# MattiaDallaCosta/JPEG-encoder-decoder

Measured on AMD Instinct MI355X. Metric: Mpixels/s encoded (device-resident BGR888 -> JFIF bytes), higher is better.
Workload: dtype int8-MFMA exact + fp64 replay (bit-exact); 1 GPU; config 3: 256 x 3840x2160 BGR888 frames per GPU, 4:2:0, Q=50, one independent JFIF per frame; frames_per_gpu=256, width=3840, height=2160, quality=50, mode=encode, pipeline=fused, parallelism=frame-parallel x1

## Files before the change

### jpeg-encoder-decoder_amd/csrc/mij_api.hip

```cpp
#include <math.h>
#include <stdarg.h>
#include <string.h>

#include <mutex>
#include <vector>

#include "mij_host.h"
#include "mij_internal.h"
#include "mij_interleave.h"
#include "mij_sampled.h"
#include "mij_ijg.h"
#include "mij_transcode.h"
#include "mijpeg.h"
#include "mij_testing.h"

namespace mij {
int k1_grid(int device, long long ntiles, int mode);
hipError_t launch_colour_lut(uint32_t *lut, hipStream_t s);
hipError_t launch_k1(const K1Args &a, int grid, int mode, hipStream_t s);
hipError_t launch_fix_blocks(const K1Args &a, hipStream_t s);
hipError_t launch_seg_dc(const EntArgs &a, hipStream_t s);
hipError_t launch_segdc_actab(const EntArgs &a, hipStream_t s);
hipError_t launch_dc_diff(int16_t *coef, const int16_t *dc, const Geom &g, int nframes,
                          const int2 *fd, hipStream_t s);
// ... 286 lines not shown
  bool assembler = false;
  std::vector<unsigned long long> band_words;
  int band_async_n = 0;
  int asm_tables_n = 0;
  int hist_zero_n = 0;
  int band_hist_zero = 0;
  int hist_zero_after = 0;
  unsigned long long *d_bound_acc = nullptr;
  int2 *d_fdims = nullptr;
  int4 *d_regions = nullptr;
  bool use_fdims = false;
  std::vector<int2> h_fdims;
  uint8_t *d_frame = nullptr;
  size_t frame_cap = 0;
  int raw_dirty = 0;
  bool keep_coefs = false;
  bool rgb = false;
  bool split = false;
  int overlap = 1;
  hipStream_t stream2 = nullptr;
  hipEvent_t ov_k1[16] = {}, ov_done = nullptr;
  bool timing = false;
  int k1_err_zero = 0;
  int opt[MIJ_OPT_COUNT] = {1, 1, 1, 0, -1, 0, 1, 0, -1};
  static constexpr int HIST = 64;
  hipEvent_t evh[HIST][MIJ_NSTAGES] = {};
  hipEvent_t *ev = evh[0];
  long long steps = 0;
  int last_frames = 0;
  int plan[MIJ_PLAN_FIELDS] = {};
  std::vector<int4> il_slot;
  long long out_cap0 = 0;
  int2 *d_il_tdims = nullptr;
  uint16_t *d_il_blk_bits = nullptr;
  uint32_t *d_il_mcu_off = nullptr, *d_il_row_bits = nullptr, *d_il_ffc = nullptr;
  uint64_t *d_il_row_pre = nullptr, *d_il_ival = nullptr, *d_il_row_off = nullptr;
  int *d_il_hdr = nullptr;
  struct DevBuf {
    void *p = nullptr;
    size_t bytes = 0;
  };
  enum { SB_PLANE, SB_ABS, SB_FR, SB_TFR, SB_TOUT, SB_BLK_BITS, SB_MCU_OFF, SB_ROW_BITS, SB_ROW_PRE, SB_IVAL,
         SB_ROW_OFF, SB_BITS, SB_HDR, SB_RAW, SB_FFC, SB_IJGQ, SB_COUNT };
  DevBuf sb[SB_COUNT];
  int samp_last = -1;
  int samp_n = 0, samp_rr = 0;
// ... 4 lines not shown
  std::vector<SampFrame> h_sfr;
  std::vector<TcFrame> h_stf;
  std::vector<TcOut> h_sto;
  int samp_test_frame = -1;
  long long samp_test_cap = 0;
};

template <class T>
static hipError_t dalloc(T **p, size_t count) {
  return hipMalloc((void **)p, count * sizeof(T) + 256);
}

static void batch_free(mij_batch *b) {
  if (!b) return;
  hipSetDevice(b->dev);
  if (b->own_stream && b->stream != b->own_stream) {
    if (b->stream && b->ev_switch && hipEventRecord(b->ev_switch, b->stream) == hipSuccess)
      hipStreamWaitEvent(b->own_stream, b->ev_switch, 0);
    b->stream = b->own_stream;
  }
  if (b->own_stream) hipStreamSynchronize(b->own_stream);
  void *ptrs[] = {b->d_tab, b->own_in ? b->d_in : nullptr, b->d_coef, b->d_dc, b->d_hist,
                  b->d_ehuf, b->d_raw, b->d_tok, b->d_tok0, b->d_seg_ntok, b->d_seg_bits, b->d_seg_off,
                  b->d_scan_bits, b->d_out_len, b->d_hc, b->d_out, b->d_err, b->d_replays,
                  b->d_dcpred, b->d_bitbase, b->d_stage, b->d_fixmask, b->d_audit, b->d_ffc, b->d_choff, b->d_scan_base,
                  b->d_seam, b->d_pack_state, b->d_pack_ticket, b->d_fdims, b->d_frame, b->d_regions, b->d_pieces,
                  b->d_bound_acc, b->d_dcx, b->d_il_tdims, b->d_il_blk_bits, b->d_il_mcu_off, b->d_il_row_bits,
                  b->d_il_ffc, b->d_il_row_pre, b->d_il_ival, b->d_il_row_off, b->d_il_hdr};
  for (void *p : ptrs)
    if (p) hipFree(p);
  for (mij_batch::DevBuf &d : b->sb)
    if (d.p) hipFree(d.p);
  for (auto &row : b->evh)
    for (auto &e : row)
      if (e) hipEventDestroy(e);
  for (auto &e : b->ov_k1)
    if (e) hipEventDestroy(e);
  if (b->ov_done) hipEventDestroy(b->ov_done);
  if (b->stream2) {
    hipStreamSynchronize(b->stream2);
    hipStreamDestroy(b->stream2);
  }
  if (b->ev_switch) hipEventDestroy(b->ev_switch);
  if (b->own_stream) hipStreamDestroy(b->own_stream);
  delete b;
}

// ... 45 lines not shown
    HIP_TRY(hipMemsetAsync(b->d_fixmask, 0, sizeof(uint16_t) * F * g.tiles_per_frame * 3, b->stream));
    HIP_TRY(dalloc(&b->d_pack_state, F * pack_stride(g)));
    HIP_TRY(dalloc(&b->d_pack_ticket, F * 3));
    HIP_TRY(dalloc(&b->d_dcx, F * 64));
    HIP_TRY(hipMemsetAsync(b->d_dcx, 0, sizeof(uint32_t) * F * 64, b->stream));
    HIP_TRY(dalloc(&b->d_seam, F * pack_stride(g)));
    HIP_TRY(dalloc(&b->d_regions, F));
  }
  HIP_TRY(dalloc(&b->d_hist, F * 4 * 257));
  HIP_TRY(dalloc(&b->d_ehuf, F * 4 * 256));
  HIP_TRY(dalloc(&b->d_raw, F * g.raw_fs));
  HIP_TRY(hipMemsetAsync(b->d_raw, 0, sizeof(uint32_t) * F * g.raw_fs, b->stream));
  HIP_TRY(dalloc(&b->d_scan_bits, F * 3));
  HIP_TRY(dalloc(&b->d_out_len, F));
  HIP_TRY(dalloc(&b->d_hc, F * 4));
  HIP_TRY(dalloc(&b->d_out, F * g.out_cap));
  HIP_TRY(dalloc(&b->d_err, F));
  HIP_TRY(dalloc(&b->d_replays, 1));
  HIP_TRY(dalloc(&b->d_ffc, F * 3 * emit_chunks(g)));
  HIP_TRY(dalloc(&b->d_choff, F * 3 * emit_chunks(g)));
  HIP_TRY(dalloc(&b->d_scan_base, F * 3));
  HIP_TRY(hipMemsetAsync(b->d_ffc, 0, sizeof(uint32_t) * F * 3 * emit_chunks(g), b->stream));
  HIP_TRY(hipMemsetAsync(b->d_replays, 0, sizeof(unsigned), b->stream));
  HIP_TRY(dalloc(&b->d_fdims, F));
  b->h_fdims.assign((size_t)F, make_int2(w, h));
  HIP_TRY(dalloc(&b->d_dcpred, F * 4));
  HIP_TRY(dalloc(&b->d_bitbase, F * 4));
  HIP_TRY(hipMemsetAsync(b->d_dcpred, 0, sizeof(int16_t) * F * 4, b->stream));
  HIP_TRY(hipMemsetAsync(b->d_bitbase, 0, sizeof(uint32_t) * F * 4, b->stream));
  b->band_words.assign((size_t)F * 3, 0);
  for (auto &row : b->evh)
    for (auto &e : row) HIP_TRY(hipEventCreate(&e));
  HIP_TRY(hipStreamSynchronize(b->stream));
  return MIJ_OK;
}

extern "C" mij_batch *mij_batch_create(int device, int width, int height, int max_frames,
                                       int quality) {
  if (!valid_dims(width, height) || max_frames < 1 || quality < 1 || quality > 100) {
    fail(MIJ_EINVAL, "batch_create: bad geometry %dx%d x%d or quality %d", width, height,
         max_frames, quality);
    return nullptr;
  }
  mij_batch *b = new mij_batch;
  if (batch_init(b, device, width, height, max_frames, quality)) {
    batch_free(b);
// ... 167 lines not shown
    a.seg_ntok += F * g.nseg;
    a.seg_bits += F * g.nseg;
    a.seg_off += F * g.nseg;
    a.scan_bits += F * 3;
    a.raw += F * g.raw_fs;
    a.hc += F * 4;
    a.out += F * g.out_cap;
    a.out_len += F;
    a.err += F;
    if (a.dc_pred) a.dc_pred += F * 4;
    if (a.bit_base) a.bit_base += F * 4;
    a.ffc += F * 3 * emit_chunks(g);
    a.choff += F * 3 * emit_chunks(g);
    a.scan_base += F * 3;
    a.pack_state += F * gpf;
    a.pack_ticket += F * 3;
    if (a.dcx) a.dcx += F * 64;
    if (a.fdims) a.fdims += F;
  }
  return a;
}

static int run_k1(mij_batch *b, int nframes, int mode, int dc_diffed = 0, int seg_dc_inline = 0, int f0 = 0,
                  bool stage_events = true, bool dc_only = false) {
  if (mode & 2) b->hist_zero_n = b->band_hist_zero = 0;
  K1Args k;
  memset(&k, 0, sizeof(k));
  k.in = b->d_in;
  k.in_fs = b->in_fs;
  k.pitch = b->pitch;
  k.nframes = nframes;
  k.g = b->g;
  k.coef = b->d_coef;
  k.dc = b->d_dc;
  k.tab = b->d_tab;
  k.replays = b->d_replays;
  k.tok = b->d_tok;
  k.tok0 = b->d_tok0;
  k.seg_ntok = b->d_seg_ntok;
  k.hist = b->d_hist;
  k.fix_mask = b->d_fixmask;
  k.audit = b->audit && mode == 1 ? b->d_audit : nullptr;
  k.rgb = b->rgb && (mode & 4) == 0;
  k.fdims = b->use_fdims ? b->d_fdims : nullptr;
  if (b->k1_err_zero) {
    k.err_zero = b->d_err;
    k.nerr_zero = b->k1_err_zero;
    b->k1_err_zero = 0;
  }
  if (f0) {
    const Geom &g = b->g;
    const long long F = f0;
    k.in += F * b->in_fs;
    k.coef += F * g.coef_fs;
    k.dc += F * g.nblk;
    k.tok += F * g.nseg * SEG_TOK;
    k.tok0 += F * g.nseg;
    k.seg_ntok += F * g.nseg;
    k.hist += F * 4 * 257;
    if (k.fdims) k.fdims += F;
  }
  static const int k1_flags = diag_env("MIJ_K1_FLAGS", 0);
  k.flags = k1_flags;
  const long long ntiles = (long long)nframes * b->g.tiles_per_frame;
  long long grid = k1_grid(b->dev, ntiles, mode);
  long long per_wg = (ntiles + grid - 1) / grid;
  if (per_wg > b->g.tiles_per_frame) per_wg = b->g.tiles_per_frame;
  grid = (ntiles + per_wg - 1) / per_wg;
  k.per_wg = (int)per_wg;
  k.dc_diffed = dc_diffed;
  k.seg_dc_inline = seg_dc_inline;
  static const bool wtime = diag_env("MIJ_K1_WTIME", 0) != 0;
  unsigned long long *d_wt = nullptr;
  const long long nw = grid * 16;
  if (wtime && (mode == 1 || mode == 2)) {
    HIP_TRY(hipMalloc(&d_wt, sizeof(unsigned long long) * K1_WTIME_WORDS * nw));
    HIP_TRY(hipMemsetAsync(d_wt, 0, sizeof(unsigned long long) * K1_WTIME_WORDS * nw, b->stream));
    k.wtime = d_wt;
  }
  k.dc_only = dc_only;
  b->plan[MIJ_PLAN_K1_MODE] = mode;
  b->plan[MIJ_PLAN_DC_ONLY] = dc_only;
  HIP_TRY(launch_k1(k, (int)grid, mode, b->stream));
  if (d_wt) {
    const int WW = K1_WTIME_WORDS;
    std::vector<unsigned long long> h(WW * nw);
    HIP_TRY(hipMemcpyAsync(h.data(), d_wt, sizeof(unsigned long long) * WW * nw, hipMemcpyDeviceToHost, b->stream));
    HIP_TRY(hipStreamSynchronize(b->stream));
    HIP_TRY(hipFree(d_wt));
    unsigned long long s0 = ~0ull, e1 = 0, e0 = ~0ull;
    double sum = 0, smin = 1e30, smax = 0, ph[5] = {0, 0, 0, 0, 0};
    long long n = 0, tiles = 0;
// ... 190 lines not shown
  if (t) HIP_TRY(hipEventRecord(b->ev[6], st));
  HIP_TRY(launch_emit(a, st));
  if (t) HIP_TRY(hipEventRecord(b->ev[7], st));
  return MIJ_OK;
}

static int encode_frames(mij_batch *b, int nframes) {
  b->plan[MIJ_PLAN_ENTROPY_CALLS] = 0;
  b->plan[MIJ_PLAN_HIST_FILL_SKIPPED] = nframes <= b->hist_zero_n;
  if (nframes > b->hist_zero_n)
    HIP_TRY(hipMemsetAsync(b->d_hist, 0, sizeof(uint32_t) * nframes * 4 * 257, b->stream));
  b->hist_zero_n = 0;
  if (b->use_fdims && b->rgb) return fail(MIJ_EINVAL, "encode: region batches read B, G, R frames");
  if (b->use_fdims)
    HIP_TRY(hipMemsetAsync(b->d_seg_ntok, 0, sizeof(uint32_t) * nframes * b->g.nseg, b->stream));
  b->k1_err_zero = nframes;
  if (b->timing) HIP_TRY(hipEventRecord(b->ev[0], b->stream));
  const bool dc_only = !b->split && !b->use_fdims && !ent_args_pack_wide(b);
  const int nsub = std::min(b->overlap, nframes);
  if (!b->split && !b->keep_coefs && nsub > 1) {
    const int per = (nframes + nsub - 1) / nsub;
    for (int k = 0, f0 = 0; f0 < nframes; k++, f0 += per) {
      const int nk = std::min(per, nframes - f0);
      if (run_k1(b, nk, 2, 0, 0, f0, false, dc_only)) return g_err;
      HIP_TRY(hipEventRecord(b->ov_k1[k], b->stream));
      HIP_TRY(hipStreamWaitEvent(b->stream2, b->ov_k1[k], 0));
      if (run_entropy(b, nk, true, false, f0, b->stream2)) return g_err;
    }
    if (b->timing)
      for (int e = 1; e <= 3; e++) HIP_TRY(hipEventRecord(b->ev[e], b->stream));
    HIP_TRY(hipEventRecord(b->ov_done, b->stream2));
    HIP_TRY(hipStreamWaitEvent(b->stream, b->ov_done, 0));
    if (b->timing)
      for (int e = 4; e < MIJ_NSTAGES; e++) HIP_TRY(hipEventRecord(b->ev[e], b->stream));
    return MIJ_OK;
  }
  if (b->split) {
    if (run_k1(b, nframes, 1)) return g_err;
    if (run_k1(b, nframes, 6, 0, 1)) return g_err;
  } else {
    if (run_k1(b, nframes, b->keep_coefs ? 3 : 2, 0, 0, 0, true, dc_only)) return g_err;
  }
  if (b->timing) HIP_TRY(hipEventRecord(b->ev[3], b->stream));
  if (run_entropy(b, nframes, !b->split, false)) return g_err;
  b->hist_zero_n = b->hist_zero_after;
  return MIJ_OK;
}

static void next_slot(mij_batch *b) {
  if (b->timing) b->ev = b->evh[b->steps++ % mij_batch::HIST];
}

extern "C" int mij_batch_encode(mij_batch *b, int nframes) {
  if (pipe_check(b, "encode")) return g_err;
  if (nframes < 1 || nframes > b->cap) return fail(MIJ_EINVAL, "encode: bad frame count");
  HIP_TRY(hipSetDevice(b->dev));
  next_slot(b);
  if (encode_frames(b, nframes)) return g_err;
  b->last_frames = nframes;
  return MIJ_OK;
}

extern "C" int mij_batch_keep_coefs(mij_batch *b, int on) {
  if (pipe_check(b, "keep_coefs")) return g_err;
// ... 558 lines not shown
    if (err[i]) return mij_frame_fail(err[i], "mij_encode_regions: region", i);
  size_t off = 0;
  for (int i = 0; i < n; i++) {
    lens[i] = len[i];
    if (off + len[i] > cap) return fail(MIJ_ENOSPC, "mij_encode_regions: need more than %zu bytes", cap);
    HIP_TRY(hipMemcpyAsync(out + off, b->d_out + (long long)i * b->g.out_cap, len[i], hipMemcpyDeviceToHost,
                           b->stream));
    off += len[i];
  }
  HIP_TRY(hipStreamSynchronize(b->stream));
  return MIJ_OK;
}

extern "C" int mij_test_last_plan(mij_batch *b, int *out, int n) {
  if (!out || n < 0) return fail(MIJ_EINVAL, "test_last_plan: bad args"), -2;
  std::unique_lock<std::mutex> l(g_mu, std::defer_lock);
  if (!b) {
    l.lock();
    b = g_rctx;
  }
  if (!b) return fail(MIJ_EINVAL, "test_last_plan: no batch"), -2;
  for (int i = 0; i < n && i < MIJ_PLAN_FIELDS; i++) out[i] = b->plan[i];
  return MIJ_PLAN_FIELDS;
}

static int band_check(mij_batch *b, int n, const char *what, bool assembling = false) {
  if (!b || n < 1 || n > b->cap) return fail(MIJ_EINVAL, "%s: bad frame count", what);
  if (!assembling && pipe_check(b, what)) return g_err;
  HIP_TRY(hipSetDevice(b->dev));
  return MIJ_OK;
}

extern "C" int mij_band_analyze(mij_batch *b, int n, int16_t *last_dc) {
  if (band_check(b, n, "band_analyze")) return g_err;
  if (!last_dc) return fail(MIJ_EINVAL, "band_analyze: null last_dc");
  HIP_TRY(hipMemsetAsync(b->d_hist, 0, sizeof(uint32_t) * n * 4 * 257, b->stream));
  HIP_TRY(hipMemsetAsync(b->d_err, 0, sizeof(int) * n, b->stream));
  if (run_k1(b, n, 2)) return g_err;
  const Geom &g = b->g;
  const long long last[3] = {g.nY - 1, g.nY + g.nC - 1, g.nY + 2LL * g.nC - 1};
  for (int c = 0; c < 3; c++)
    HIP_TRY(hipMemcpy2DAsync(last_dc + c, 3 * sizeof(int16_t), b->d_dc + last[c], sizeof(int16_t) * g.nblk,
                             sizeof(int16_t), n, hipMemcpyDeviceToHost, b->stream));
  HIP_TRY(hipStreamSynchronize(b->stream));
  return MIJ_OK;
}
// ... 1064 lines not shown
```

### jpeg-encoder-decoder_amd/csrc/mij_internal.h

```cpp
#pragma once
#include <hip/hip_runtime.h>
#include <stddef.h>
#include <stdint.h>

#include "mij_divmagic.h"

namespace mij {

constexpr int TILE_W = 128;
constexpr int TILE_H = 16;
constexpr int LDS_BLK = 80;
constexpr int LDS_WAVE = 48 * LDS_BLK;
constexpr int LUT_WORDS = 1024;
constexpr int DCTIE_WORDS = 33;

constexpr int FERR_TABLE = 1;
constexpr int FERR_OVERFLOW = 2;
constexpr int FERR_ASSEMBLY = 3;
constexpr int OPT_TEST_FAULT_TICKET = 7;
constexpr int FERR_SPIN = 4;
constexpr unsigned long long SPIN_TICKS = 200000000ull;

constexpr int MAX_BLOCK_TOK = 65;
constexpr int SEG_TOK = 16 * MAX_BLOCK_TOK;
// ... 86 lines not shown
  int nframes;
  Geom g;
  int16_t *coef;
  int16_t *dc;
  const Tables *tab;
  unsigned int *replays;
  int flags;
  int per_wg;
  int dc_diffed;
  int seg_dc_inline;
  const int16_t *dc_pred;
  uint32_t *tok;
  uint32_t *tok0;
  uint32_t *seg_ntok;
  uint32_t *hist;
  uint16_t *fix_mask;
  unsigned long long *wtime;
  int rgb;
  const int2 *fdims;
  uint16_t *audit;
  int *err_zero;
  int nerr_zero;
  int dc_only;
};
constexpr int K1_WTIME_WORDS = 8;
constexpr int K1F_NO_LUT = 1, K1F_NO_REPLAY = 2, K1F_NO_COLOUR = 4, K1F_NO_DCT = 8,
              K1F_NO_STORE = 16, K1F_NO_QUANT = 32, K1F_NO_MFMA = 64,
              K1F_LINEAR_STORE = 128, K1F_PLAIN_STORE = 256,
              K1F_NO_HIST = 512, K1F_NO_TOKSTORE = 1024,
              K1F_EXTRA_LDS = 2048, K1F_NO_EMIT = 4096, K1F_NO_ACLOOP = 8192,
              K1F_NO_DMAWAIT = 16384,
              K1F_REPLAY_NO_FP64 = 32768,
              K1F_COUNT_PASSES = 65536,
              K1F_COUNT_LUMA = 131072;

struct EntArgs {
  Geom g;
  int nframes;
  const int16_t *coef;
  const int16_t *dc;
  uint32_t *hist;
  const uint32_t *ehuf;
  uint32_t *tok;
  uint32_t *tok0;
  const uint32_t *seg_ntok;
  uint32_t *seg_bits;
  uint64_t *seg_off;
// ... 50 lines not shown
```

### jpeg-encoder-decoder_amd/csrc/mij_kernels.hip

```cpp
#include <stdlib.h>

#include "mij_internal.h"
#include "mij_headers.h"
#include "mij_colour_f64.h"

namespace mij {

typedef int v4i __attribute__((ext_vector_type(4)));
typedef unsigned u4v __attribute__((ext_vector_type(4)));
typedef unsigned short us2 __attribute__((ext_vector_type(2)));

__constant__ int c_zigzag[64] = {
    0,  1,  8,  16, 9,  2,  3,  10, 17, 24, 32, 25, 18, 11, 4,  5,
    12, 19, 26, 33, 40, 48, 41, 34, 27, 20, 13, 6,  7,  14, 21, 28,
    35, 42, 49, 56, 57, 50, 43, 36, 29, 22, 15, 23, 30, 37, 44, 51,
    58, 59, 52, 45, 38, 31, 39, 46, 53, 60, 61, 54, 47, 55, 62, 63};

#define SQRT1_2 0.70710678118654752440

__device__ __forceinline__ void wave_lds_sync() {
  __builtin_amdgcn_fence(__ATOMIC_RELEASE, "wavefront");
  __builtin_amdgcn_wave_barrier();
  __builtin_amdgcn_fence(__ATOMIC_ACQUIRE, "wavefront");
}
// ... 481 lines not shown
      const uint32_t bef = __builtin_amdgcn_ubfe(Mhi, 0u, (uint32_t)zz);
      uint32_t lz;
      asm("v_ffbh_u32 %0, %1" : "=v"(lz) : "v"(bef));
      token(32 + zz, rank_lo1 + __popc(bef), (int)min(lz, (uint32_t)(63 - zp_lo)));
    }
  }
  wave_lds_sync();
}

constexpr int K1M_COEF_OUT = 1;
constexpr int K1M_TOK_OUT = 2;
constexpr int K1M_COEF_IN = 4;
constexpr int K1M_RGB = 8;
constexpr int K1M_REGIONS = 16;
constexpr int K1M_AUDIT = 32;
constexpr int K1M_FLOOR = 64;
constexpr int k1_base(int mode) { return mode & ~(K1M_RGB | K1M_REGIONS | K1M_AUDIT | K1M_FLOOR); }

template <int MODE>
constexpr bool k1_wide() { return k1_base(MODE) == K1M_COEF_OUT || k1_base(MODE) == K1M_TOK_OUT; }
template <int MODE>
constexpr int k1_waves() {
  return k1_wide<MODE>() ? 12 : 4;
}

template <int MODE>
__global__ __launch_bounds__(64 * k1_waves<MODE>(), k1_wide<MODE>() ? 1 : 2) void k_mcu_dct(K1Args a) {
  constexpr bool PIX = !(MODE & K1M_COEF_IN);
  constexpr bool TOK = MODE & K1M_TOK_OUT;
  constexpr int NW = k1_waves<MODE>();
  constexpr int NT = 64 * NW;
  constexpr bool DEFER = k1_base(MODE) == K1M_COEF_OUT;
  constexpr bool RGB = MODE & K1M_RGB;
  constexpr bool REG = MODE & K1M_REGIONS;
  constexpr bool AUDIT = MODE & K1M_AUDIT;
  constexpr bool FLOOR = MODE & K1M_FLOOR;
  const int2 *const fdims = REG ? a.fdims : nullptr;
  __shared__ __attribute__((aligned(16))) uint8_t s_raw[PIX ? NW : 1][TILE_RAW];
  __shared__ __attribute__((aligned(16))) uint8_t s_tile[PIX ? NW : 1][LDS_WAVE];
  __shared__ __attribute__((aligned(16))) int4 s_A[PIX ? 12 * 64 : 1];
  __shared__ __attribute__((aligned(16))) float s_fac[2][64];
  __shared__ float s_inv8q[2];
  __shared__ uint32_t s_dctie[2][DCTIE_WORDS];
  constexpr bool LUT_LDS = PIX && !(TOK && NW >= 8);
  __shared__ uint32_t s_lut[LUT_LDS ? 3 * LUT_WORDS : 1];
  __shared__ double s_cos[64];
  __shared__ uint8_t s_zz[64];
  __shared__ int s_qint[2][64];
  __shared__ __attribute__((aligned(16))) int s_czl[PIX ? 64 : 1];
  __shared__ __attribute__((aligned(16))) int16_t s_st[TOK ? NW : 1][64][16];
  constexpr int HREP = PIX ? 1 : 4;
  __shared__ uint32_t s_hac[TOK ? 2 : 1][2][HREP][256];
  __shared__ uint32_t s_hdc[TOK ? 2 : 1][2][HREP][16];
  __shared__ int s_next;

  const Tables *__restrict__ T = a.tab;
#ifdef MIJ_K1_DIAG
  const int kflags = a.flags;
#else
  constexpr int kflags = 0;
#endif
  if (threadIdx.x < 64) {
    s_cos[threadIdx.x] = T->cosd[threadIdx.x];
    s_zz[threadIdx.x] = (uint8_t)c_zigzag[threadIdx.x];
  }
  if (TOK) {
    for (int i = threadIdx.x; i < 2 * 2 * HREP * 256; i += NT) (&s_hac[0][0][0][0])[i] = 0;
    for (int i = threadIdx.x; i < 2 * 2 * HREP * 16; i += NT) (&s_hdc[0][0][0][0])[i] = 0;
  }
  if (threadIdx.x < 128) s_qint[threadIdx.x >> 6][threadIdx.x & 63] = T->qint[threadIdx.x >> 6][threadIdx.x & 63];
  if (threadIdx.x < 2) s_inv8q[threadIdx.x] = 1.0f / (float)(8 * T->qint[threadIdx.x][0]);
  if (PIX && threadIdx.x < 64) s_czl[threadIdx.x] = T->czl[threadIdx.x];
  if (threadIdx.x < 2 * DCTIE_WORDS) (&s_dctie[0][0])[threadIdx.x] = (&T->dctie[0][0])[threadIdx.x];
  if (PIX) {
    for (int i = threadIdx.x; i < 12 * 64; i += NT) s_A[i] = T->mfma_a[i];
    if (LUT_LDS)
      for (int i = threadIdx.x; i < 3 * LUT_WORDS; i += NT) s_lut[i] = (&T->lut[0][0])[i];
  }
  const uint32_t *__restrict__ lut = LUT_LDS ? (const uint32_t *)s_lut : &T->lut[0][0];
  for (int i = threadIdx.x; i < 128; i += NT) {
    s_fac[i >> 6][i & 63] = T->qfac[i >> 6][i & 63];
  }
  if (threadIdx.x == 0) s_next = (int)blockIdx.x * a.per_wg + NW;
  if (blockIdx.x == 0)
    for (int i = threadIdx.x; i < a.nerr_zero; i += NT) a.err_zero[i] = 0;
  __syncthreads();

  const int lane = threadIdx.x & 63;
  const int wave = __builtin_amdgcn_readfirstlane(threadIdx.x >> 6);
  uint8_t *L = s_tile[PIX ? wave : 0];
  const int g = lane >> 4, bcol = lane & 15;
  const int c4 = lane & 31, pr = lane >> 5;
  const uint32_t kq = (uint32_t)T->kq[g];
  const int q_dc[2] = {T->qint[0][0], T->qint[1][0]};
  const bool cz_on = PIX && !AUDIT && T->cz_on;
  const Geom &G = a.g;
  const int bw = G.w >> 3, mw = G.w >> 4;
  const int ntiles = a.nframes * G.tiles_per_frame;
  const int t0 = (int)blockIdx.x * a.per_wg;
  const int f0 = t0 / G.tiles_per_frame;
  const int tend = min(ntiles, t0 + a.per_wg);
  int t = t0 + wave;
  auto skip_outside = [&](int &tt) {
    bool ok;
    while (tt < tend && (tile_pos_r(G, fdims, tt, ok), !ok)) {
      int v = 0;
      if (lane == 0) v = atomicAdd(&s_next, 1);
      tt = __builtin_amdgcn_readfirstlane(v);
    }
  };
  auto tpos = [&](int tt) {
    bool ok;
    return REG ? tile_pos_r(G, fdims, tt, ok) : tile_pos(G, tt);
  };
  if (REG) skip_outside(t);
#ifdef MIJ_K1_DIAG
  const unsigned long long w_t0 = __builtin_amdgcn_s_memrealtime();
  int w_ntiles = 0;
  unsigned long long ph[5] = {0, 0, 0, 0, 0}, tph = __builtin_amdgcn_s_memtime();
#define K1_PHASE(k)                                                  \
  do {                                                               \
    const unsigned long long tn_ = __builtin_amdgcn_s_memtime();     \
    ph[k] += tn_ - tph;                                              \
    tph = tn_;                                                       \
  } while (0)
#else
#define K1_PHASE(k)
#endif
  uint32_t nrep = 0;
  if (t < tend) {
    uint8_t *raw = s_raw[PIX ? wave : 0];
    TilePos p = tpos(t);
    const DmaOff doff = dma_offsets(a.pitch, lane);
    if (PIX) issue_tile_dma(a, p, lane, raw, doff);
    auto load_coefs = [&](const TilePos &pp, u4v (&dst)[PIX ? 1 : 3][2]) {
#pragma unroll
      for (int nt = 0; nt < 3; nt++) {
        bool valid;
        long long blk;
        const FGeom fg = frame_geom(G, fdims, pp.f);
        const int bwf = REG ? fg.bw : bw, mwf = REG ? fg.mw : mw;
        const int nYf = REG ? fg.nY : G.nY, nCf = REG ? fg.nC : G.nC;
        if (nt < 2) {
          const int bx = pp.tx * 16 + bcol;
          valid = bx < bwf;
          blk = (long long)(2 * pp.ty + nt) * bwf + bx;
        } else {
          const int mx = pp.tx * 8 + (bcol & 7);
          valid = mx < mwf;
          blk = nYf + (bcol >= 8 ? nCf : 0) + (long long)pp.ty * mwf + mx;
        }
        dst[PIX ? 0 : nt][0] = dst[PIX ? 0 : nt][1] = u4v{0, 0, 0, 0};
        if (valid) {
          const int16_t *src = a.coef + (long long)pp.f * G.coef_fs + blk * 64 + 16 * g;
          dst[PIX ? 0 : nt][0] = *(const u4v *)src;
          dst[PIX ? 0 : nt][1] = *(const u4v *)(src + 8);
        }
      }
    };
    u4v cnext[PIX ? 1 : 3][2];
    if (!PIX) load_coefs(p, cnext);
    bool first = true;
    for (;;) {
      TilePos pn = p;
      int tn = 0;
      if (lane == 0) tn = atomicAdd(&s_next, 1);
      tn = __builtin_amdgcn_readfirstlane(tn);
      uint32_t fl_w = 0;
      if (PIX) {
        K1_PHASE(3);
        if (first || (kflags & (K1F_NO_DCT | K1F_NO_STORE)))
          dma_wait();
        else if (DEFER)
          dma_wait_behind_stores();
        K1_PHASE(0);
        if (!(kflags & K1F_NO_COLOUR) && !FLOOR) colour_stage<RGB, !LUT_LDS>(raw, L, c4, pr, lut, !(kflags & K1F_NO_LUT));
        if (FLOOR) fl_w = ((const uint32_t *)raw)[lane];
        wave_lds_sync();
        K1_PHASE(1);
        if (REG) skip_outside(tn);
        if (tn < tend) {
          pn = tpos(tn);
          issue_tile_dma(a, pn, lane, raw, doff);
        }
        K1_PHASE(2);
      } else {
        if (REG) skip_outside(tn);
        if (tn < tend) pn = tpos(tn);
      }

      const bool do_dct = !(kflags & K1F_NO_DCT);
      auto dct_digit = [&](const int d, v4i (&acc)[4], const v4i Bf) {
#pragma unroll
        for (int m = 0; m < 4; m++) {
          const int4 F = s_A[(3 * m + d) * 64 + lane];
#ifdef MIJ_K1_DIAG
          if (kflags & K1F_EXTRA_LDS) {
            v4i dummy;
            asm volatile("ds_read_b128 %0, %1\n\ts_waitcnt lgkmcnt(0)" : "=v"(dummy) : "v"((uint32_t)(uintptr_t)(lds_void_t *)&s_A[(3 * m + d) * 64 + lane]) : "memory");
          }
#endif
          const v4i Fv = {F.x, F.y, F.z, F.w};
          v4i c;
          if (d == 0) {
// ... 90 lines not shown
              __builtin_nontemporal_store(s1, (u4v *)(lin + 512));
            } else {
              *(u4v *)dst = s0;
              *(u4v *)(dst + 8) = s1;
            }
          } else {
            u4v d1, d2;
#pragma unroll
            for (int k = 0; k < 4; k++) {
              d1[k] = (uint32_t)__builtin_amdgcn_update_dpp((int)s0[k], (int)s1[k], 0x128, 0xF, 0xC, false);
              d2[k] = (uint32_t)__builtin_amdgcn_update_dpp((int)s1[k], (int)s0[k], 0x128, 0xF, 0x3, false);
            }
            const int off = 16 * g + 8 * (bcol >> 3);
            int b1, b2;
            const bool v1 = block_at(nt, bcol & 7, b1), v2 = block_at(nt, bcol | 8, b2);
            int16_t *const p1 = fcoef + (long long)b1 * 64 + off;
            if (v1) __builtin_nontemporal_store(d1, (u4v *)p1);
            if (v1 || v2) __builtin_nontemporal_store(v2 ? d2 : d1, (u4v *)(v2 ? fcoef + (long long)b2 * 64 + off : p1));
          }
        }
        if (PIX && valid && g == 0) a.dc[(long long)p.f * G.nblk + blk] = (int16_t)o[0];
        if (TOK && !(kflags & K1F_NO_EMIT)) {
          const long long fs = (long long)p.f * G.nseg + seg;
          const int slot = p.f - f0;
          int pred0 = 0;
          const bool first_pred = !PIX && a.seg_dc_inline;
          if (first_pred && valid && g == 0 && (comp == 1 ? (bcol & 7) : bcol) == 0) {
            const FGeom fg = frame_geom(G, fdims, p.f);
            const int nYf = REG ? fg.nY : G.nY, nCf = REG ? fg.nC : G.nC;
            const int cstart = comp == 0 ? 0 : (bcol >= 8 ? nYf + nCf : nYf);
            pred0 = blk == cstart ? (a.dc_pred ? (int)a.dc_pred[p.f * 4 + (comp == 0 ? 0 : (bcol >= 8 ? 2 : 1))] : 0)
                                  : (int)a.dc[(long long)p.f * G.nblk + blk - 1];
          }
          emit_tokens(o, lane, g, bcol, valid, comp == 1, !PIX && a.dc_diffed, first_pred, pred0,
                      a.tok + (long long)p.f * G.nseg * SEG_TOK, (uint32_t)seg * SEG_TOK, a.tok0 + fs,
                      a.seg_ntok + fs, s_hdc[TOK ? slot : 0][comp][bcol & (HREP - 1)],
                      s_hac[TOK ? slot : 0][comp][bcol & (HREP - 1)],
                      s_st[TOK ? wave : 0], kflags, acz, PIX && !REG && a.dc_only);
        }
      };
      if (FLOOR) {
#pragma unroll
        for (int nt = 0; nt < 3; nt++) {
          int o[16];
#pragma unroll
          for (int k = 0; k < 16; k++) o[k] = (int)(fl_w >> k) & 0xFF;
          finish(nt, o, false);
// ... 215 lines not shown
                    }
                  }
                }
                wave_lds_sync();
              }
            }
          }
          if (nt == 0 && !DEFER && !(kflags & K1F_NO_DMAWAIT)) dma_wait();
          K1_PHASE(3);
          finish(nt, o, false);
          K1_PHASE(4);
        }
      } else if (!PIX) {
#pragma unroll
        for (int nt = 0; nt < 3; nt++) {
          int o[16];
          finish(nt, o, false);
        }
      }
      if (PIX) wave_lds_sync();
#ifdef MIJ_K1_DIAG
      w_ntiles++;
#endif
      if (tn >= tend) break;
      p = pn;
      t = tn;
      first = false;
    }
  }
  if (__ballot(nrep != 0)) {
    const uint32_t tot = wave_scan64(nrep);
    if (lane == 63) atomicAdd(a.replays, tot);
  }
#ifdef MIJ_K1_DIAG
  if (a.wtime && lane == 0) {
    unsigned long long *w = a.wtime + K1_WTIME_WORDS * ((long long)blockIdx.x * NW + wave);
    w[0] = w_t0;
    w[1] = __builtin_amdgcn_s_memrealtime();
    w[2] = (unsigned long long)w_ntiles;
    for (int k = 0; k < 5; k++) w[3 + k] = ph[k];
  }
#endif
  if (TOK) {
    __syncthreads();
    for (int i = threadIdx.x; i < 2 * 2 * 256; i += NT) {
      const int slot = i >> 9, tb = (i >> 8) & 1, sym = i & 255;
      uint32_t v = 0;
#pragma unroll
      for (int c = 0; c < HREP; c++) v += s_hac[slot][tb][c][sym];
      if (v && f0 + slot < a.nframes)
        atomicAdd(&a.hist[((long long)(f0 + slot) * 4 + (tb ? 3 : 1)) * 257 + sym], v);
    }
    if (threadIdx.x < 64) {
      const int slot = threadIdx.x >> 5, tb = (threadIdx.x >> 4) & 1, sym = threadIdx.x & 15;
      uint32_t v = 0;
#pragma unroll
      for (int c = 0; c < HREP; c++) v += s_hdc[slot][tb][c][sym];
      if (v && f0 + slot < a.nframes)
        atomicAdd(&a.hist[((long long)(f0 + slot) * 4 + (tb ? 2 : 0)) * 257 + sym], v);
    }
  }
}


__device__ __forceinline__ int y_ref(const uint8_t *px, int ib, int ir) { return y_f64(px[ir], px[1], px[ib]); }
__device__ __forceinline__ int cb_ref(const uint8_t *px, int ib, int ir) { return cb_f64(px[ir], px[1], px[ib]); }
__device__ __forceinline__ int cr_ref(const uint8_t *px, int ib, int ir) { return cr_f64(px[ir], px[1], px[ib]); }

__global__ __launch_bounds__(256) void k_fix_blocks(K1Args a) {
  __shared__ __attribute__((aligned(8))) uint8_t s_px[4][64];
  __shared__ double s_inner[4][64];
  __shared__ double s_cos[64];
  __shared__ int s_q[2][64];
  const Tables *__restrict__ T = a.tab;
  if (threadIdx.x < 64) s_cos[threadIdx.x] = T->cosd[threadIdx.x];
  if (threadIdx.x < 128) s_q[threadIdx.x >> 6][threadIdx.x & 63] = T->qint[threadIdx.x >> 6][threadIdx.x & 63];
  __syncthreads();
  const int lane = threadIdx.x & 63, wave = threadIdx.x >> 6;
  const Geom G = a.g;
  const int x = lane & 7, y = lane >> 3;
  const int rz = c_zigzag[lane], v = rz >> 3, u = rz & 7;
  const int ib = a.rgb ? 2 : 0, ir = 2 - ib;
// ... 2543 lines not shown
```

### jpeg-encoder-decoder_amd/csrc/mij_testing.h

```cpp
#ifndef MIJ_TESTING_H
#define MIJ_TESTING_H
#include "mijpeg.h"
#ifdef __cplusplus
extern "C" {
#endif
int mij_test_stale_ticket(mij_batch *b, int v);

enum {
  MIJ_PLAN_NFRAMES = 0,
  MIJ_PLAN_F0,
  MIJ_PLAN_ENTROPY_CALLS,
  MIJ_PLAN_DC_LAST,
  MIJ_PLAN_ACTAB,
  MIJ_PLAN_TABLES,
  MIJ_PLAN_SEGDC,
  MIJ_PLAN_SEAM,
  MIJ_PLAN_FF_PACK,
  MIJ_PLAN_SEAM_IN_SCAN,
  MIJ_PLAN_EMIT_SLOTS,
  MIJ_PLAN_PACK_LS_LUMA,
  MIJ_PLAN_PACK_LS_CHROMA,
  MIJ_PLAN_PACK_WIDE,
  MIJ_PLAN_HIST_FILL_SKIPPED,
  MIJ_PLAN_K1_MODE,
  MIJ_PLAN_DC_ONLY,
  MIJ_PLAN_FIELDS
};
int mij_test_last_plan(mij_batch *b, int *out, int n);

int mij_test_sampled_out_cap(mij_batch *b, int frame, long long cap);
int mij_test_prog_mapping(mij_decoder *d, int mapping);

#ifdef __cplusplus
}
#endif
#endif
```

### jpeg-encoder-decoder_amd/mijpeg.py

```python
from __future__ import annotations

import ctypes as C
import math
import os

import numpy as np

HERE = os.path.dirname(os.path.abspath(__file__))
LIB_PATH = os.environ.get("MIJ_LIB") or os.path.join(HERE, "libmijpeg.so")

EXPORTS = [
    "rgb_to_dct", "init_huffman", "write_jpg",
    "mij_set_input_stride", "mij_set_quality", "mij_last_error", "mij_strerror", "mij_last_message",
    "mij_max_jpg_bytes", "mij_encode",
    "mij_batch_create", "mij_batch_destroy", "mij_batch_upload", "mij_batch_set_input",
    "mij_batch_encode", "mij_batch_keep_coefs", "mij_batch_set_split", "mij_batch_set_overlap", "mij_batch_set_option", "mij_batch_get_option", "mij_batch_dct", "mij_batch_pattern_floor", "mij_batch_sync", "mij_batch_output",
    "mij_batch_lengths", "mij_batch_coefs", "mij_batch_tables", "mij_batch_set_timing",
    "mij_batch_stage_ms", "mij_batch_stage_history", "mij_batch_token_count", "mij_batch_geometry", "mij_batch_replays", "mij_batch_stream", "mij_batch_set_stream", "mij_batch_audit", "mij_batch_build_tables",
    "mij_band_analyze", "mij_band_histograms", "mij_band_tables", "mij_band_pack", "mij_band_words",
    "mij_assemble_begin", "mij_assemble_words", "mij_assemble_end",
    "mij_band_words_all", "mij_assemble_pieces", "mij_assembler_create",
    "mij_band_analyze_async", "mij_band_histograms_async", "mij_band_tables_async", "mij_band_pack_async",
    "mij_band_words_async", "mij_assemble_tables_async", "mij_assemble_async",
    "mij_band_stuff_async", "mij_assemble_stuffed_async", "mij_copy_to_host_async",
# ... 38 lines not shown
        ("code_len", C.c_int * 257),
        ("next", C.c_int * 257),
        ("code_len_freq", C.c_int * 32),
        ("sym_sorted", C.c_int * 256),
        ("sym_code_len", C.c_int * 256),
        ("sym_code", C.c_int * 256),
    ]


class Area(C.Structure):
    _fields_ = [("x", C.c_int), ("y", C.c_int), ("w", C.c_int), ("h", C.c_int)]


class MijError(RuntimeError):
    pass


OPTIONS = {"seam": 0, "ff_pack": 1, "actab": 2, "segdc_fused": 3, "pack_wide": 4, "emit_slots": 5,
           "overlap_prio": 6, "pack_segs": 8}


PLAN_FIELDS = ["nframes", "f0", "entropy_calls", "dc_last", "actab", "tables", "segdc", "seam", "ff_pack",
               "seam_in_scan", "emit_slots", "pack_ls_luma", "pack_ls_chroma", "pack_wide",
               "hist_fill_skipped", "k1_mode", "dc_only"]


_lib = None


def load() -> C.CDLL:
    global _lib
    if _lib is not None:
        return _lib
    if not os.path.exists(LIB_PATH):
        raise MijError(f"{LIB_PATH} missing: build it with `make -C {HERE}` "
                       "(there is no CPU fallback)")
    lib = C.CDLL(LIB_PATH)
    p, i, sz = C.c_void_p, C.c_int, C.c_size_t
    lib.rgb_to_dct.argtypes = [p, p, p, p, Area]
    lib.rgb_to_dct.restype = None
    lib.init_huffman.argtypes = [p, p, p, Area, p, p]
    lib.init_huffman.restype = None
    lib.write_jpg.argtypes = [p, p, p, p, p, Area, p, p]
    lib.write_jpg.restype = sz
    lib.mij_set_input_stride.argtypes = [i]
    lib.mij_set_quality.argtypes = [i]
    lib.mij_last_error.restype = i
# ... 487 lines not shown
        out = np.zeros((bw * bh, 64), np.int16)
        _check(self.lib.mij_batch_sampled_component(self.h_, frame, comp, _ptr(out), out.size), "sampled_component")
        return out

    def upload(self, frames_bgr: np.ndarray, first: int = 0) -> None:
        frames_bgr = np.ascontiguousarray(frames_bgr, np.uint8)
        n = frames_bgr.shape[0] if frames_bgr.ndim == 4 else 1
        _check(self.lib.mij_batch_upload(self.h_, _ptr(frames_bgr), first, n), "upload")
        if self.fdims is not None:
            dims = list(self.fdims) + [(self.w, self.h)] * max(0, self.max_frames - len(self.fdims))
            dims[first:first + n] = [(self.w, self.h)] * n
            self.fdims = None if all(d == (self.w, self.h) for d in dims) else dims

    def set_input(self, dev_ptr: int, frame_stride: int, pitch: int) -> None:
        _check(self.lib.mij_batch_set_input(self.h_, dev_ptr, frame_stride, pitch), "set_input")
        self.fdims = None

    def encode(self, n: int) -> None:
        _check(self.lib.mij_batch_encode(self.h_, n), "encode")

    def last_plan(self) -> dict:
        return _last_plan(self.h_)

    def dct(self, n: int) -> None:
        _check(self.lib.mij_batch_dct(self.h_, n), "dct")

    def pattern_floor(self, n: int) -> None:
        _check(self.lib.mij_batch_pattern_floor(self.h_, n), "pattern_floor")

    def sync(self) -> None:
        _check(self.lib.mij_batch_sync(self.h_), "sync")

    def output(self, frame: int) -> bytes:
        n = C.c_size_t(0)
        _check(self.lib.mij_batch_output(self.h_, frame, None, 0, C.byref(n)), "output")
        buf = np.zeros(max(n.value, 1), np.uint8)
        _check(self.lib.mij_batch_output(self.h_, frame, _ptr(buf), buf.size, C.byref(n)),
               "output")
        return buf[:n.value].tobytes()

    def lengths(self, n: int) -> np.ndarray:
        arr = (C.c_size_t * n)()
        _check(self.lib.mij_batch_lengths(self.h_, arr, n), "lengths")
        return np.array(arr[:], np.int64)

    def coefs(self, frame: int, diffed: bool = True):
# ... 954 lines not shown
```

Before: 594,000 Mpixels/s.

## Let K1 workgroups span frame boundaries and steal tail tiles from a shared pool

Removes the cap that kept each K1 workgroup's tile range inside one frame. Each workgroup now holds two LDS histogram slots keyed by frame, and a slot is flushed to global memory when the wave moves to a new frame. A slice of the tail tiles is also placed in a global work pool that workgroups claim in chunks through atomics, so load stays balanced at the end of the kernel. The aim is to cut tail imbalance and fix grid-size effects, at the cost of more atomics, spin-waits with timeout error paths, and more complex histogram accounting.

```diff
diff --git a/jpeg-encoder-decoder_amd/csrc/mij_api.hip b/jpeg-encoder-decoder_amd/csrc/mij_api.hip
--- a/jpeg-encoder-decoder_amd/csrc/mij_api.hip
+++ b/jpeg-encoder-decoder_amd/csrc/mij_api.hip
@@ -332,6 +332,8 @@
   hipEvent_t ov_k1[16] = {}, ov_done = nullptr;
   bool timing = false;
   int k1_err_zero = 0;
+  unsigned *d_k1_pool = nullptr;
+  int k1_test_grid = 0, k1_test_pool_den = 0, k1_test_pool_chunk = 0;
   int opt[MIJ_OPT_COUNT] = {1, 1, 1, 0, -1, 0, 1, 0, -1};
   static constexpr int HIST = 64;
   hipEvent_t evh[HIST][MIJ_NSTAGES] = {};
@@ -382,7 +384,7 @@
   if (b->own_stream) hipStreamSynchronize(b->own_stream);
   void *ptrs[] = {b->d_tab, b->own_in ? b->d_in : nullptr, b->d_coef, b->d_dc, b->d_hist,
                   b->d_ehuf, b->d_raw, b->d_tok, b->d_tok0, b->d_seg_ntok, b->d_seg_bits, b->d_seg_off,
-                  b->d_scan_bits, b->d_out_len, b->d_hc, b->d_out, b->d_err, b->d_replays,
+                  b->d_scan_bits, b->d_out_len, b->d_hc, b->d_out, b->d_err, b->d_replays, b->d_k1_pool,
                   b->d_dcpred, b->d_bitbase, b->d_stage, b->d_fixmask, b->d_audit, b->d_ffc, b->d_choff, b->d_scan_base,
                   b->d_seam, b->d_pack_state, b->d_pack_ticket, b->d_fdims, b->d_frame, b->d_regions, b->d_pieces,
                   b->d_bound_acc, b->d_dcx, b->d_il_tdims, b->d_il_blk_bits, b->d_il_mcu_off, b->d_il_row_bits,
@@ -474,6 +476,8 @@
   HIP_TRY(dalloc(&b->d_scan_base, F * 3));
   HIP_TRY(hipMemsetAsync(b->d_ffc, 0, sizeof(uint32_t) * F * 3 * emit_chunks(g), b->stream));
   HIP_TRY(hipMemsetAsync(b->d_replays, 0, sizeof(unsigned), b->stream));
+  HIP_TRY(dalloc(&b->d_k1_pool, 2));
+  HIP_TRY(hipMemsetAsync(b->d_k1_pool, 0, 2 * sizeof(unsigned), b->stream));
   HIP_TRY(dalloc(&b->d_fdims, F));
   b->h_fdims.assign((size_t)F, make_int2(w, h));
   HIP_TRY(dalloc(&b->d_dcpred, F * 4));
@@ -687,7 +691,7 @@
 }
 
 static int run_k1(mij_batch *b, int nframes, int mode, int dc_diffed = 0, int seg_dc_inline = 0, int f0 = 0,
-                  bool stage_events = true, bool dc_only = false) {
+                  bool stage_events = true, bool dc_only = false, bool span = false) {
   if (mode & 2) b->hist_zero_n = b->band_hist_zero = 0;
   K1Args k;
   memset(&k, 0, sizeof(k));
@@ -730,9 +734,39 @@
   const long long ntiles = (long long)nframes * b->g.tiles_per_frame;
   long long grid = k1_grid(b->dev, ntiles, mode);
   long long per_wg = (ntiles + grid - 1) / grid;
-  if (per_wg > b->g.tiles_per_frame) per_wg = b->g.tiles_per_frame;
-  grid = (ntiles + per_wg - 1) / per_wg;
+  k.err = b->d_err + f0;
+  k.pool_ctr = b->d_k1_pool;
+  static const int k1_pool_den = diag_env("MIJ_K1_POOL_DEN", K1_POOL_DEN);
+  static const int k1_pool_chunk = diag_env("MIJ_K1_POOL_CHUNK", K1_POOL_CHUNK);
+  long long own = ntiles;
+  if (span && !b->use_fdims) {
+    if (b->k1_test_grid > 0) grid = std::min<long long>(b->k1_test_grid, ntiles);
+    const int den = b->k1_test_grid > 0 ? b->k1_test_pool_den : k1_pool_den;
+    const int chunk = b->k1_test_grid > 0 ? b->k1_test_pool_chunk : k1_pool_chunk;
+    if (den > 0 && chunk > 0 && chunk <= K1_POOL_CHUNK_MAX && ntiles / den / chunk <= K1_POOL_CHUNKS_MAX &&
+        (b->k1_test_grid > 0 || ntiles / den >= grid * 16)) {
+      k.pool_chunk = chunk;
+      k.pool_chunks = (int)(ntiles / den / chunk);
+      own = ntiles - (long long)k.pool_chunks * chunk;
+      k.pool_t0 = (int)own;
+      if (!k.pool_chunks) k.pool_chunk = 0;
+    }
+    per_wg = std::max(1ll, (own + grid - 1) / grid);
+    if (!k.pool_chunks) grid = (ntiles + per_wg - 1) / per_wg;
+  } else {
+    if (per_wg > b->g.tiles_per_frame) per_wg = b->g.tiles_per_frame;
+    grid = (ntiles + per_wg - 1) / per_wg;
+  }
   k.per_wg = (int)per_wg;
+  int widest = 0;
+  for (long long t0 = 0; t0 < own; t0 += per_wg) {
+    const long long t1 = std::min(own, t0 + per_wg) - 1;
+    widest = std::max(widest, (int)(t1 / b->g.tiles_per_frame - t0 / b->g.tiles_per_frame) + 1);
+  }
+  b->plan[MIJ_PLAN_K1_GRID] = (int)grid;
+  b->plan[MIJ_PLAN_K1_SPAN_FRAMES] = widest;
+  b->plan[MIJ_PLAN_K1_POOL_CHUNKS] = k.pool_chunks;
+  b->plan[MIJ_PLAN_K1_POOL_CHUNK] = k.pool_chunk;
   k.dc_diffed = dc_diffed;
   k.seg_dc_inline = seg_dc_inline;
   static const bool wtime = diag_env("MIJ_K1_WTIME", 0) != 0;
@@ -969,7 +1003,7 @@
     const int per = (nframes + nsub - 1) / nsub;
     for (int k = 0, f0 = 0; f0 < nframes; k++, f0 += per) {
       const int nk = std::min(per, nframes - f0);
-      if (run_k1(b, nk, 2, 0, 0, f0, false, dc_only)) return g_err;
+      if (run_k1(b, nk, 2, 0, 0, f0, false, dc_only, true)) return g_err;
       HIP_TRY(hipEventRecord(b->ov_k1[k], b->stream));
       HIP_TRY(hipStreamWaitEvent(b->stream2, b->ov_k1[k], 0));
       if (run_entropy(b, nk, true, false, f0, b->stream2)) return g_err;
@@ -986,7 +1020,7 @@
     if (run_k1(b, nframes, 1)) return g_err;
     if (run_k1(b, nframes, 6, 0, 1)) return g_err;
   } else {
-    if (run_k1(b, nframes, b->keep_coefs ? 3 : 2, 0, 0, 0, true, dc_only)) return g_err;
+    if (run_k1(b, nframes, b->keep_coefs ? 3 : 2, 0, 0, 0, true, dc_only, true)) return g_err;
   }
   if (b->timing) HIP_TRY(hipEventRecord(b->ev[3], b->stream));
   if (run_entropy(b, nframes, !b->split, false)) return g_err;
@@ -1591,6 +1625,16 @@
   if (!b) return fail(MIJ_EINVAL, "test_last_plan: no batch"), -2;
   for (int i = 0; i < n && i < MIJ_PLAN_FIELDS; i++) out[i] = b->plan[i];
   return MIJ_PLAN_FIELDS;
+}
+
+extern "C" int mij_test_k1_partition(mij_batch *b, int grid, int pool_den, int pool_chunk) {
+  if (!b || grid < 0 || grid > 65535 || pool_den < 0 || pool_chunk < 0 || pool_chunk > K1_POOL_CHUNK_MAX ||
+      (pool_den > 0 && pool_chunk < 1))
+    return fail(MIJ_EINVAL, "test_k1_partition: bad args"), -2;
+  b->k1_test_grid = grid;
+  b->k1_test_pool_den = grid ? pool_den : 0;
+  b->k1_test_pool_chunk = grid ? pool_chunk : 0;
+  return 0;
 }
 
 static int band_check(mij_batch *b, int n, const char *what, bool assembling = false) {
diff --git a/jpeg-encoder-decoder_amd/csrc/mij_internal.h b/jpeg-encoder-decoder_amd/csrc/mij_internal.h
--- a/jpeg-encoder-decoder_amd/csrc/mij_internal.h
+++ b/jpeg-encoder-decoder_amd/csrc/mij_internal.h
@@ -132,7 +132,12 @@
   int *err_zero;
   int nerr_zero;
   int dc_only;
-};
+  int *err;
+  int pool_t0, pool_chunk, pool_chunks;
+  unsigned *pool_ctr;
+};
+constexpr int K1_POOL_DEN = 64, K1_POOL_CHUNK = 24;
+constexpr int K1_POOL_CHUNK_MAX = 255, K1_POOL_CHUNKS_MAX = 0xFFFFFF;
 constexpr int K1_WTIME_WORDS = 8;
 constexpr int K1F_NO_LUT = 1, K1F_NO_REPLAY = 2, K1F_NO_COLOUR = 4, K1F_NO_DCT = 8,
               K1F_NO_STORE = 16, K1F_NO_QUANT = 32, K1F_NO_MFMA = 64,
diff --git a/jpeg-encoder-decoder_amd/csrc/mij_kernels.hip b/jpeg-encoder-decoder_amd/csrc/mij_kernels.hip
--- a/jpeg-encoder-decoder_amd/csrc/mij_kernels.hip
+++ b/jpeg-encoder-decoder_amd/csrc/mij_kernels.hip
@@ -527,6 +527,88 @@
 template <int MODE>
 constexpr int k1_waves() {
   return k1_wide<MODE>() ? 12 : 4;
+}
+
+struct K1Slots {
+  uint32_t w[2];
+  uint32_t pool;
+};
+constexpr uint32_t K1_SLOT_FLUSH = 0xFF;
+constexpr uint32_t K1_POOL_EMPTY = 0u, K1_POOL_BUSY = 0xFFFFFFFEu, K1_POOL_DONE = 0xFFFFFFFFu;
+constexpr int K1_NO_TILE = 0x7FFFFFFF;
+#define K1_WG __HIP_MEMORY_SCOPE_WORKGROUP
+
+__device__ __forceinline__ int k1_lane() {
+  int l = (int)__builtin_amdgcn_mbcnt_hi(~0u, __builtin_amdgcn_mbcnt_lo(~0u, 0u));
+  asm volatile("" : "+v"(l));
+  return l;
+}
+
+template <class Flush>
+__device__ __forceinline__ int k1_slot_acquire(K1Slots &S, int f, Flush &&flush) {
+  const unsigned long long t_wait = __builtin_amdgcn_s_memrealtime();
+  const uint32_t tag = (uint32_t)(f + 1) << 8;
+  for (;;) {
+    const uint32_t w0 = __builtin_amdgcn_readfirstlane(__hip_atomic_load(&S.w[0], __ATOMIC_RELAXED, K1_WG));
+    const uint32_t w1 = __builtin_amdgcn_readfirstlane(__hip_atomic_load(&S.w[1], __ATOMIC_RELAXED, K1_WG));
+    int i = (w0 & ~0xFFu) == tag ? 0 : ((w1 & ~0xFFu) == tag ? 1 : -1);
+    const bool take = i < 0;
+    if (take) i = (w0 & 0xFF) == 0 ? 0 : ((w1 & 0xFF) == 0 ? 1 : -1);
+    const uint32_t w = i == 1 ? w1 : w0;
+    bool wait = i < 0 || (w & 0xFF) == K1_SLOT_FLUSH;
+    if (!wait) {
+      int ok = 0;
+      if (k1_lane() == 0) {
+        uint32_t seen = w;
+        ok = __hip_atomic_compare_exchange_strong(&S.w[i], &seen, take ? tag | K1_SLOT_FLUSH : w + 1, __ATOMIC_ACQUIRE,
+                                                  __ATOMIC_RELAXED, K1_WG);
+      }
+      if (__builtin_amdgcn_readfirstlane(ok)) {
+        if (take) {
+          if (w >> 8) flush(i, (int)(w >> 8) - 1);
+          if (k1_lane() == 0) __hip_atomic_store(&S.w[i], tag | 1u, __ATOMIC_RELEASE, K1_WG);
+        }
+        return i;
+      }
+    }
+    if (__builtin_amdgcn_s_memrealtime() - t_wait > SPIN_TICKS) return -1;
+    if (wait) __builtin_amdgcn_s_sleep(8);
+  }
+}
+__device__ __forceinline__ void k1_slot_release(K1Slots &S, int i) {
+  if (k1_lane() == 0) __hip_atomic_fetch_sub(&S.w[i], 1u, __ATOMIC_RELEASE, K1_WG);
+}
+
+__device__ __forceinline__ int k1_pool_claim(K1Slots &Sk, const K1Args &a) {
+  int zero = 0;
+  asm volatile("" : "+s"(zero));
+  uint32_t *const pool = &Sk.pool + zero;
+  const unsigned long long t_wait = __builtin_amdgcn_s_memrealtime();
+  for (;;) {
+    const uint32_t cur = __builtin_amdgcn_readfirstlane(__hip_atomic_load(pool, __ATOMIC_RELAXED, K1_WG));
+    if (cur == K1_POOL_DONE) return K1_NO_TILE;
+    if (cur != K1_POOL_BUSY) {
+      const uint32_t left = cur & 0xFF;
+      int ok = 0;
+      if (k1_lane() == 0) {
+        uint32_t seen = cur;
+        ok = __hip_atomic_compare_exchange_strong(pool, &seen, left ? cur - 1 : K1_POOL_BUSY, __ATOMIC_RELAXED,
+                                                  __ATOMIC_RELAXED, K1_WG);
+      }
+      if (__builtin_amdgcn_readfirstlane(ok)) {
+        if (left) return a.pool_t0 + (int)(cur >> 8) * a.pool_chunk + (a.pool_chunk - (int)left);
+        uint32_t k = 0;
+        if (k1_lane() == 0) k = __hip_atomic_fetch_add(&a.pool_ctr[0], 1u, __ATOMIC_RELAXED, __HIP_MEMORY_SCOPE_AGENT);
+        k = __builtin_amdgcn_readfirstlane(k);
+        const bool more = k < (uint32_t)a.pool_chunks;
+        if (k1_lane() == 0)
+          __hip_atomic_store(pool, more ? k << 8 | (uint32_t)(a.pool_chunk - 1) : K1_POOL_DONE, __ATOMIC_RELAXED, K1_WG);
+        return more ? a.pool_t0 + (int)k * a.pool_chunk : K1_NO_TILE;
+      }
+    }
+    if (__builtin_amdgcn_s_memrealtime() - t_wait > SPIN_TICKS) return K1_NO_TILE;
+    if (cur == K1_POOL_BUSY) __builtin_amdgcn_s_sleep(8);
+  }
 }
 
 template <int MODE>
@@ -558,6 +640,8 @@
   __shared__ uint32_t s_hac[TOK ? 2 : 1][2][HREP][256];
   __shared__ uint32_t s_hdc[TOK ? 2 : 1][2][HREP][16];
   __shared__ int s_next;
+  constexpr bool SPAN = TOK && PIX && !REG;
+  __shared__ K1Slots s_fs;
 
   const Tables *__restrict__ T = a.tab;
 #ifdef MIJ_K1_DIAG
@@ -587,6 +671,10 @@
     s_fac[i >> 6][i & 63] = T->qfac[i >> 6][i & 63];
   }
   if (threadIdx.x == 0) s_next = (int)blockIdx.x * a.per_wg + NW;
+  if (SPAN && threadIdx.x == 0) {
+    s_fs.w[0] = s_fs.w[1] = 0;
+    s_fs.pool = a.pool_chunks ? K1_POOL_EMPTY : K1_POOL_DONE;
+  }
   if (blockIdx.x == 0)
     for (int i = threadIdx.x; i < a.nerr_zero; i += NT) a.err_zero[i] = 0;
   __syncthreads();
@@ -604,8 +692,25 @@
   const int ntiles = a.nframes * G.tiles_per_frame;
   const int t0 = (int)blockIdx.x * a.per_wg;
   const int f0 = t0 / G.tiles_per_frame;
-  const int tend = min(ntiles, t0 + a.per_wg);
+  const int tend = min(SPAN && a.pool_chunks ? a.pool_t0 : ntiles, t0 + a.per_wg);
+  auto is_tile = [&](int tt) { return SPAN ? tt != K1_NO_TILE : tt < tend; };
   int t = t0 + wave;
+  if (SPAN && t >= tend) t = k1_pool_claim(s_fs, a);
+  auto flush_slot = [&](int i, int f) {
+    uint32_t *const h = a.hist + (long long)f * 4 * 257;
+    uint32_t *const hac = &s_hac[TOK ? i : 0][0][0][0], *const hdc = &s_hdc[TOK ? i : 0][0][0][0];
+    const int ln = k1_lane();
+#pragma unroll 1
+    for (int k = ln; k < 2 * 256; k += 64) {
+      const uint32_t v = __hip_atomic_exchange(&hac[k], 0u, __ATOMIC_RELAXED, K1_WG);
+      if (v) atomicAdd(&h[257 + k + (k >> 8) * 258], v);
+    }
+    if (ln < 32) {
+      const uint32_t v = __hip_atomic_exchange(&hdc[ln], 0u, __ATOMIC_RELAXED, K1_WG);
+      if (v) atomicAdd(&h[(ln >> 4) * 514 + (ln & 15)], v);
+    }
+  };
+  int slot = 0;
   auto skip_outside = [&](int &tt) {
     bool ok;
     while (tt < tend && (tile_pos_r(G, fdims, tt, ok), !ok)) {
@@ -633,11 +738,17 @@
 #define K1_PHASE(k)
 #endif
   uint32_t nrep = 0;
-  if (t < tend) {
+  if (is_tile(t)) {
     uint8_t *raw = s_raw[PIX ? wave : 0];
     TilePos p = tpos(t);
     const DmaOff doff = dma_offsets(a.pitch, lane);
     if (PIX) issue_tile_dma(a, p, lane, raw, doff);
+    if (SPAN) slot = k1_slot_acquire(s_fs, __builtin_amdgcn_readfirstlane(p.f), flush_slot);
+    auto slot_failed = [&](int f) {
+      if (k1_lane() == 0) a.err[f] = FERR_SPIN;
+      dma_wait();
+    };
+    if (SPAN && slot < 0) slot_failed(p.f);
     auto load_coefs = [&](const TilePos &pp, u4v (&dst)[PIX ? 1 : 3][2]) {
 #pragma unroll
       for (int nt = 0; nt < 3; nt++) {
@@ -666,11 +777,12 @@
     u4v cnext[PIX ? 1 : 3][2];
     if (!PIX) load_coefs(p, cnext);
     bool first = true;
-    for (;;) {
+    while (!SPAN || slot >= 0) {
       TilePos pn = p;
       int tn = 0;
       if (lane == 0) tn = atomicAdd(&s_next, 1);
       tn = __builtin_amdgcn_readfirstlane(tn);
+      if (__builtin_expect(SPAN && tn >= tend, 0)) tn = k1_pool_claim(s_fs, a);
       uint32_t fl_w = 0;
       if (PIX) {
         K1_PHASE(3);
@@ -684,7 +796,7 @@
         wave_lds_sync();
         K1_PHASE(1);
         if (REG) skip_outside(tn);
-        if (tn < tend) {
+        if (is_tile(tn)) {
           pn = tpos(tn);
           issue_tile_dma(a, pn, lane, raw, doff);
         }
@@ -821,7 +933,7 @@
         if (PIX && valid && g == 0) a.dc[(long long)p.f * G.nblk + blk] = (int16_t)o[0];
         if (TOK && !(kflags & K1F_NO_EMIT)) {
           const long long fs = (long long)p.f * G.nseg + seg;
-          const int slot = p.f - f0;
+          if (!SPAN) slot = p.f - f0;
           int pred0 = 0;
           const bool first_pred = !PIX && a.seg_dc_inline;
           if (first_pred && valid && g == 0 && (comp == 1 ? (bcol & 7) : bcol) == 0) {
@@ -1083,11 +1195,17 @@
 #ifdef MIJ_K1_DIAG
       w_ntiles++;
 #endif
-      if (tn >= tend) break;
+      if (!is_tile(tn)) break;
+      if (SPAN && __builtin_amdgcn_readfirstlane(pn.f) != __builtin_amdgcn_readfirstlane(p.f)) {
+        k1_slot_release(s_fs, slot);
+        slot = k1_slot_acquire(s_fs, __builtin_amdgcn_readfirstlane(pn.f), flush_slot);
+        if (slot < 0) slot_failed(pn.f);
+      }
       p = pn;
       t = tn;
       first = false;
     }
+    if (SPAN && slot >= 0) k1_slot_release(s_fs, slot);
   }
   if (__ballot(nrep != 0)) {
     const uint32_t tot = wave_scan64(nrep);
@@ -1104,21 +1222,27 @@
 #endif
   if (TOK) {
     __syncthreads();
+    auto sf = [&](int i) { return SPAN ? (int)(s_fs.w[i] >> 8) - 1 : f0 + i; };
     for (int i = threadIdx.x; i < 2 * 2 * 256; i += NT) {
       const int slot = i >> 9, tb = (i >> 8) & 1, sym = i & 255;
       uint32_t v = 0;
 #pragma unroll
       for (int c = 0; c < HREP; c++) v += s_hac[slot][tb][c][sym];
-      if (v && f0 + slot < a.nframes)
-        atomicAdd(&a.hist[((long long)(f0 + slot) * 4 + (tb ? 3 : 1)) * 257 + sym], v);
+      if (v && sf(slot) >= 0 && sf(slot) < a.nframes)
+        atomicAdd(&a.hist[((long long)sf(slot) * 4 + (tb ? 3 : 1)) * 257 + sym], v);
     }
     if (threadIdx.x < 64) {
       const int slot = threadIdx.x >> 5, tb = (threadIdx.x >> 4) & 1, sym = threadIdx.x & 15;
       uint32_t v = 0;
 #pragma unroll
       for (int c = 0; c < HREP; c++) v += s_hdc[slot][tb][c][sym];
-      if (v && f0 + slot < a.nframes)
-        atomicAdd(&a.hist[((long long)(f0 + slot) * 4 + (tb ? 2 : 0)) * 257 + sym], v);
+      if (v && sf(slot) >= 0 && sf(slot) < a.nframes)
+        atomicAdd(&a.hist[((long long)sf(slot) * 4 + (tb ? 2 : 0)) * 257 + sym], v);
+    }
+    if (SPAN && a.pool_chunks && threadIdx.x == 0 &&
+        __hip_atomic_fetch_add(&a.pool_ctr[1], 1u, __ATOMIC_RELAXED, __HIP_MEMORY_SCOPE_AGENT) == gridDim.x - 1) {
+      __hip_atomic_store(&a.pool_ctr[0], 0u, __ATOMIC_RELAXED, __HIP_MEMORY_SCOPE_AGENT);
+      __hip_atomic_store(&a.pool_ctr[1], 0u, __ATOMIC_RELAXED, __HIP_MEMORY_SCOPE_AGENT);
     }
   }
 }
diff --git a/jpeg-encoder-decoder_amd/csrc/mij_testing.h b/jpeg-encoder-decoder_amd/csrc/mij_testing.h
--- a/jpeg-encoder-decoder_amd/csrc/mij_testing.h
+++ b/jpeg-encoder-decoder_amd/csrc/mij_testing.h
@@ -24,9 +24,15 @@
   MIJ_PLAN_HIST_FILL_SKIPPED,
   MIJ_PLAN_K1_MODE,
   MIJ_PLAN_DC_ONLY,
+  MIJ_PLAN_K1_SPAN_FRAMES,
+  MIJ_PLAN_K1_POOL_CHUNKS,
+  MIJ_PLAN_K1_POOL_CHUNK,
+  MIJ_PLAN_K1_GRID,
   MIJ_PLAN_FIELDS
 };
 int mij_test_last_plan(mij_batch *b, int *out, int n);
+
+int mij_test_k1_partition(mij_batch *b, int grid, int pool_den, int pool_chunk);
 
 int mij_test_sampled_out_cap(mij_batch *b, int frame, long long cap);
 int mij_test_prog_mapping(mij_decoder *d, int mapping);
diff --git a/jpeg-encoder-decoder_amd/mijpeg.py b/jpeg-encoder-decoder_amd/mijpeg.py
--- a/jpeg-encoder-decoder_amd/mijpeg.py
+++ b/jpeg-encoder-decoder_amd/mijpeg.py
@@ -84,7 +84,8 @@
 
 PLAN_FIELDS = ["nframes", "f0", "entropy_calls", "dc_last", "actab", "tables", "segdc", "seam", "ff_pack",
                "seam_in_scan", "emit_slots", "pack_ls_luma", "pack_ls_chroma", "pack_wide",
-               "hist_fill_skipped", "k1_mode", "dc_only"]
+               "hist_fill_skipped", "k1_mode", "dc_only", "k1_span_frames", "k1_pool_chunks", "k1_pool_chunk",
+               "k1_grid"]
 
 
 _lib = None
@@ -618,6 +619,12 @@
     def last_plan(self) -> dict:
         return _last_plan(self.h_)
 
+    def test_k1_partition(self, grid: int, pool_den: int = 0, pool_chunk: int = 0) -> None:
+        fn = self.lib.mij_test_k1_partition
+        fn.argtypes, fn.restype = [C.c_void_p, C.c_int, C.c_int, C.c_int], C.c_int
+        if fn(self.h_, grid, pool_den, pool_chunk) != 0:
+            raise MijError(f"mij_test_k1_partition({grid}, {pool_den}, {pool_chunk}) refused")
+
     def dct(self, n: int) -> None:
         _check(self.lib.mij_batch_dct(self.h_, n), "dct")
 
```

Result: no change. 599,300 Mpixels/s, median of 6 (+0.9%).
